# JaehaKim97/EDTR

Measured on AMD Instinct MI355X. Metric: restored 512x512 images/sec @ 4 denoise steps, higher is better.
Workload: dtype bf16; 1 GPU; EDTR-det s4 (sd21): vae_encode + q_sample(t=200) + 4 x (ControlNet+UNet) + vae_decode, batch 8/GPU of 512x512; global_batch=8, image_size=512, denoise_steps=4, parallelism=batch-sharded x1, graphs=True, batches_in_flight=2, precision=fast

## Files before the change

edtr_amd/csrc/lin320.hip:

```cpp
#include <stdlib.h>
#include <type_traits>
#include "common.h"

namespace {

constexpr int LK = 320;
constexpr int LKS = LK / 16;
constexpr int LBM = 128;
constexpr int LCH = 32;
constexpr int LCHB = LCH * LK * 2;
constexpr int LPITCH = 272;
constexpr int LVPITCH = 144;
constexpr int LSTGB = 64 * LVPITCH;
constexpr int L_STG = 2 * LCHB;
constexpr int L_CV = L_STG + 4 * LSTGB;
constexpr int L_LDS = L_CV + 4096;
static_assert(LSTGB >= 32 * LPITCH && 2 * L_LDS <= 160 * 1024, "LDS budget");

template <int N> __device__ __forceinline__ void lwait() {
    static_assert(N == 0 || N == 4 || N == 5 || N == 9, "lwait");
    if constexpr (N == 0) asm volatile("s_waitcnt vmcnt(0)" ::: "memory");
    else if constexpr (N == 4) asm volatile("s_waitcnt vmcnt(4)" ::: "memory");
    else if constexpr (N == 5) asm volatile("s_waitcnt vmcnt(5)" ::: "memory");
    else asm volatile("s_waitcnt vmcnt(9)" ::: "memory");
// ... 186 lines not shown
        case 2: return go(&lin320_kernel<T, true, false, false>);
        case 3: return go(&lin320_kernel<T, true, true, false>);
        case 4: return go(&lin320_kernel<T, false, false, true>);
        default: return go(&lin320_kernel<T, false, true, true>);
    }
}

int check_lin320(const edtr_lin320_params& p) {
    if (!p.x || !p.w || !p.out) return EDTR_E_NULL;
    if (p.dtype != EDTR_BF16 && p.dtype != EDTR_F16) return EDTR_E_DTYPE;
    if (p.K != LK || p.M <= 0 || p.N <= 0) return EDTR_E_SHAPE;
    if ((p.M % LBM) || (p.N % 64) || p.N > 1024) return EDTR_E_UNSUPPORTED;
    if (p.ldx < LK || (p.residual && p.ldr < p.N)) return EDTR_E_SHAPE;
    if ((p.ldx & 7) || (p.ldo & 7) || (p.residual && (p.ldr & 7))) return EDTR_E_ALIGN;
    if (!aligned16(p.x) || !aligned16(p.w) || !aligned16(p.out) || (p.residual && !aligned16(p.residual)) || (p.cvec && !aligned16(p.cvec))) return EDTR_E_ALIGN;
    if (p.x == p.out) return EDTR_E_UNSUPPORTED;
    if (p.gn_table) {
        if (p.ln || p.rows_per_image <= 0 || (p.rows_per_image % LBM) || (p.M % p.rows_per_image)) return EDTR_E_UNSUPPORTED;
        if (!aligned16(p.gn_table)) return EDTR_E_ALIGN;
    }
    if (p.vt_out) {
        if (p.residual || p.vt_col0 <= 0 || p.vt_col0 >= p.N || (p.vt_col0 & 63) || p.rows_per_image <= 0 || (p.rows_per_image & 31) ||
            (p.M % p.rows_per_image) || p.vt_ld < p.rows_per_image)
            return EDTR_E_UNSUPPORTED;
        if ((p.vt_ld & 7) || !aligned16(p.vt_out)) return EDTR_E_ALIGN;
        if (p.ldo < p.vt_col0) return EDTR_E_SHAPE;
    } else if (p.ldo < p.N) {
        return EDTR_E_SHAPE;
    }
    if ((int64_t)p.N * LK * 2 >= 0xF0000000LL) return EDTR_E_UNSUPPORTED;
    return EDTR_OK;
}

}

extern "C" int edtr_lin320(const edtr_lin320_params* pp, edtr_stream_t stream) {
    if (!pp) return EDTR_E_NULL;
    if (int e = check_lin320(*pp)) return e;
    hipStream_t s = static_cast<hipStream_t>(stream);
    return pp->dtype == EDTR_BF16 ? launch_lin320<BF16>(*pp, s) : launch_lin320<F16>(*pp, s);
}

extern "C" int edtr_lin320_plan(const edtr_lin320_params* pp) {
    if (!pp) return EDTR_E_NULL;
    return check_lin320(*pp);
}
```

edtr_amd/engine.py:

```python
from __future__ import annotations

import collections
import ctypes as ct
import math
import os
from dataclasses import dataclass
from typing import Dict, List, Optional, Sequence, Tuple

import torch

from . import lib as L
from . import ops
from .ops import Rec, round_up


class Arena:

    ALIGN = 256

    def __init__(self, device: torch.device, chunk_bytes: int = 1 << 28):
        self.device = device
        self.chunk_bytes = chunk_bytes
        self.chunks: List[torch.Tensor] = []
        self.free_lists: List[List[List[int]]] = []
# ... 225 lines not shown
            npad = packed.shape[0]
            c1 = packed[:, : w.shape[1]].float().sum(dim=1).contiguous()
            c2 = ops.pad_bias(w @ beta, npad).contiguous()
            self.cache[key] = (packed, ops.pad_bias(b, npad) if b is not None else None, c1, c2)
        packed, b, c1, c2 = self.cache[key]
        return packed, b, c1, c2

    def ffn(self, w1name: str, b1name: str, w2name: str, b2name: str, ln_prefix: str):
        key = ("ffn", w1name, w2name, ln_prefix)
        if key not in self.cache:
            w1p, b1p, c1, c2 = self.ln_fold("geglu", [w1name], [b1name], ln_prefix)
            cst = ops.pack_ffn_constants(c2 + b1p)
            w2p = ops.pack_ffn_w2(self._p(w2name).reshape(self.params[w2name].shape[0], -1), self.dtype)
            self.cache[key] = (w1p, w2p, cst, self._p(b2name).reshape(-1).contiguous())
        return self.cache[key]

    def lin320(self, names: Sequence[str], biases, ln_prefix: Optional[str], alpha: float, vt_col0: Optional[int] = None, vt_alpha: float = 1.0):
        names = tuple(names)
        key = ("lin320", names, tuple(biases) if biases else None, ln_prefix, float(alpha), vt_col0, float(vt_alpha))
        if key not in self.cache:
            w = torch.cat([self._p(n).reshape(self.params[n].shape[0], -1) for n in names], dim=0)
            cvec = None
            if biases:
                cvec = torch.cat([self._p(bn).reshape(-1) if bn else torch.zeros(self.params[n].shape[0], device=self.device)
                                  for n, bn in zip(names, biases)]).float()
            if ln_prefix is not None:
                gamma, beta = self._p(ln_prefix + "weight").reshape(-1), self._p(ln_prefix + "bias").reshape(-1)
                shift = float(alpha) * (w @ beta)
                if vt_col0 is not None:
                    shift[vt_col0:] *= float(vt_alpha) / float(alpha)
                cvec = shift if cvec is None else cvec + shift
                w = w * gamma[None, :]
            self.cache[key] = (ops.pack_lin320_w(w, self.dtype), cvec.contiguous() if cvec is not None else None)
        return self.cache[key]

    def raw(self, name: str) -> torch.Tensor:
        key = ("raw", name)
        if key not in self.cache:
            self.cache[key] = self._p(name).contiguous()
        return self.cache[key]

    def geglu(self, wname: str, bname: str):
        n, k = self.shape_of(wname)[0], self.shape_of(wname)[1]

        def build(parts):
            w = self._p(wname)
            perm = ops.geglu_perm(w.shape[0] // 2).to(self.device)
            return ops.pack_linear_weight(w[perm], self.dtype, parts=parts)

        ref = WRef(self, ("geglu", wname), build, (round_up(n, 8), round_up(k, 8)))
        key = ("geglu.bias", bname)
        if key not in self.cache:
            b = self._p(bname)
            self.cache[key] = b[ops.geglu_perm(b.shape[0] // 2).to(self.device)].contiguous()
        return ref, self.cache[key]

    def tensors(self) -> List[torch.Tensor]:
        out: List[torch.Tensor] = []
        seen = set()
        stores = [self] + [self._siblings[k] for k in sorted(self._siblings, key=str)]
        for st in stores:
            for key in sorted(st.cache, key=repr):
                val = st.cache[key]
                for t in (val if isinstance(val, (tuple, list)) else (val,)):
                    if isinstance(t, torch.Tensor) and t.data_ptr() not in seen:
                        seen.add(t.data_ptr())
# ... 450 lines not shown
        self.arena.free(tmp)
        return qk, vt, N

    def conv(self, x: Act, prefix: str, *, taps=9, stride=1, pad_tl=1, ups=False, rowvec=None, residual=None,
             out=None, out_f32=False, alpha=1.0, name=None, stats=False, feeds=None, mirror=False, gnp_into=None) -> Act:
        name = name or ("conv3x3" if taps == 9 else "conv1x1")
        w, bias = self.store.conv(prefix, cin_pad=x.C, bias_scale=alpha)
        N = w.shape[0]
        if taps == 9:
            LH, LW = (x.H * 2, x.W * 2) if ups else (x.H, x.W)
            pad_br = 1
            OH = (LH + pad_tl + pad_br - 3) // stride + 1
            OW = (LW + pad_tl + pad_br - 3) // stride + 1
            spatial = (x.H, x.W, OH, OW, stride, pad_tl, pad_tl, int(ups))
        else:
            OH, OW, spatial = x.H, x.W, None
        M = x.B * OH * OW
        parts = self.parts_for(name, M, N, taps * x.C)
        if parts == ops.PARTS_2W and (taps != 1 or x.C % 64):
            parts = 3
        if x.gn_in is not None:
            img8_ = taps == 9 and stride == 1 and pad_tl == 1 and not ups and (x.H, x.W) == (8, 8) and x.C % 64 == 0
            fusable = (taps == 9 and stride == 1 and pad_tl == 1 and not ups and not self.invariant
                       and (not self.hp or (x.t.dtype == self.dtype and parts == 1))
                       and ops.gn_in_conv_ok(x.B, x.H, x.W, x.C, N, ops.choose_splitk(M, N, taps * x.C, img8=img8_)[1], x.ld))
            if not fusable:
                if x.gn_apply is None:
                    raise RuntimeError(f"{name}: a deferred GroupNorm reached a convolution that cannot apply it")
                xn = x.gn_apply()
                y = self.conv(xn, prefix, taps=taps, stride=stride, pad_tl=pad_tl, ups=ups, rowvec=rowvec, residual=residual, out=out,
                              out_f32=out_f32, alpha=alpha, name=name, stats=stats, feeds=feeds, mirror=mirror, gnp_into=gnp_into)
                self.free(xn)
                return y
        a, tmp = x.t, None
        if self.hp:
            a, tmp, parts = self._operand(x.t, x.rows, x.C, parts)
            out_f32 = True if out is None else out.dtype == torch.float32
            if out is None and self.branch16 and feeds and self.feeds_parts(feeds, M) == 1:
                out_f32 = False
        Ce = ops.k_mult(parts) * x.C
        subpix = (ups and taps == 9 and stride == 1 and pad_tl == 1 and not self.invariant
                  and ops.subpixel_ok(x.H, x.W, Ce, N, x.B, a.stride(0)))
        if subpix:
            w, bias = self.store.conv_subpixel(prefix, cin_pad=x.C, bias_scale=alpha)
            spatial = spatial[:7] + (2,)
        wt = self._w(w, parts)
        m16 = None
        if out is None:
            out = self.new(M, N, torch.float32 if out_f32 else (self.dtype if self.hp else None))
            if mirror and self.mirrors_on and out_f32:
                m16 = self.add_mirror(out)
        elif self.mirrors_on and out_f32:
            m16 = self.mirror_view(out)
        img8 = taps == 9 and stride == 1 and pad_tl == 1 and not ups and (x.H, x.W) == (8, 8) and Ce % 64 == 0
        tile, splitk = ops.choose_splitk(M, N, taps * Ce, img8=img8)
        if self.invariant:
            tile, splitk = ops.invariant_tile(Ce, 0), 1
        if subpix:
            tile, splitk = 16, 1
        if x.gn_in is not None:
            if (taps != 9 or stride != 1 or pad_tl != 1 or ups or (self.hp and (a.dtype != self.dtype or parts != 1 or a is not x.t))
                    or not ops.gn_in_conv_ok(x.B, x.H, x.W, x.C, N, splitk, x.ld)):
                raise RuntimeError(f"{name}: a deferred GroupNorm reached a convolution that cannot apply it")
            tile = 0
        ws = self.arena.alloc((splitk * M * N,), torch.float32) if splitk > 1 else None
        gnp, gn_slot, into = None, 128, None
        self.gnp_into_done = False
        if stats and (self.hp or not out_f32) and out.stride(0) == N and ops.gn_fusable(M, N, Ce, OH * OW, splitk=splitk, invariant=self.invariant):
            gn_slot = ops.gn_slot_rows(OH * OW) if splitk > 1 else 128
            gnp = self.arena.alloc((M // gn_slot, N, 2), torch.float32)
        elif gnp_into is not None and not out_f32:
            into = self._gnp_into_args(gnp_into, M, N, Ce, OH * OW, splitk)
            self.gnp_into_done = into is not None
        res32 = residual is not None and residual.dtype == torch.float32
        self.prog.add(ops.make_igemm(
            dtype=self.dtype, a1=a, w=wt, out=out, taps=taps, M=M, N=N, C1=Ce, ld1=a.stride(0), ldw=wt.stride(0),
            ldc=out.stride(0), spatial=spatial, bias_n=bias, rowvec=rowvec,
            rowvec_ld=rowvec.stride(0) if rowvec is not None else 0, rows_per_image=OH * OW, residual=residual,
            ldr=residual.stride(0) if residual is not None else 0, residual_f32=res32, out_f32=out_f32, alpha=alpha, tile=tile,
            splitk=splitk, workspace=ws, name=name,
            **(into if into is not None else dict(gn_partial=gnp, gn_slot_rows=gn_slot if splitk > 1 else 0)),
            w_phase_stride=(N * wt.stride(0)) if subpix else 0,
            out16=m16, a_wrap=x.C if parts == ops.PARTS_2W else 0, a_gn=x.gn_in, a_gn_silu=x.gn_silu))
        self.arena.free(ws)
        self.arena.free(tmp)
        return Act(out, x.B, OH, OW, N, gnp, gn_slot=gn_slot)

    def conv128_out(self, x: Act, prefix: str, out_nchw: torch.Tensor, n_valid: int, alpha: float = 1.0, name="vae.conv_out") -> None:
        key = ("conv128_out", prefix, alpha)
        if key not in self.store.cache:
            w = self.store._p(prefix + "weight")
            self.store.cache[key] = (ops.pack_conv128_out_weight(w, self.dtype), ops.pad_bias(self.store._p(prefix + "bias") * alpha, 32))
        w, b = self.store.cache[key]
        self.prog.add(ops.make_conv128_out(dtype=self.dtype, x=x.t, ldx=x.ld, w=w, bias=b, out=out_nchw, B=x.B, H=x.H, W=x.W, n_valid=n_valid,
                                           gn_table=x.gn_in, alpha=alpha, name=name))

    def _gn_recs(self, x: Act, prefix: str, eps: float, silu: bool, sums: Optional[torch.Tensor], y: torch.Tensor,
                 sums_zeroed: bool = False, parts: int = 1, partial=None):
        gamma, beta = self.store.vec(prefix + "weight", x.C), self.store.vec(prefix + "bias", x.C)
        c_real = self.store.params[prefix + "weight"].numel()
        if c_real != x.C:
            raise ValueError(f"GroupNorm {prefix}: activation has {x.C} channels, parameter has {c_real}")
        in32 = x.t.dtype == torch.float32
        return ops.make_gn(dtype=(self.op_fmt(parts) if in32 else self.dtype) if self.hp else self.io, x=x.t, ldx=x.ld, B=x.B, HW=x.H * x.W, C=x.C,
                           sums=sums, gamma=gamma, beta=beta, eps=eps, silu=silu, y=y, ldy=y.stride(0), sums_zeroed=sums_zeroed,
                           partial=partial, tiles_per_image=x.gn_tiles)

    def _norm_out(self, rows: int, C: int, parts: int):
        if self.hp:
            t = self.arena.alloc((rows, parts * C), self.dtype)
            return t, OpN(t, C, parts)
        y = self.new(rows, C)
        return y, y

    def gn_deferrable(self, x: Act, conv_n: int, feeds=None) -> bool:
        if not conv_n or self.invariant or x.t.dtype == torch.float32:
            return False
        if self.hp and (conv_n < 0 or x.t.dtype != self.dtype or feeds is None or self.feeds_parts(feeds, x.rows) != 1
                        or os.environ.get("EDTR_GN_IN_CONV_HP", "1") == "0"):
            return False
# ... 230 lines not shown
```

edtr_amd/lib.py:

```python
from __future__ import annotations

import ctypes as C
import os
from typing import Optional

HERE = os.path.dirname(os.path.abspath(__file__))
LIB_PATH = os.environ.get("EDTR_AMD_LIB") or os.path.join(HERE, "libedtr_hip.so")

BF16, F16, F32_SPLIT, F32_H1, F32_H2, F32_H3 = 0, 1, 2, 3, 4, 5
ACT_NONE, ACT_GEGLU, ACT_SILU, ACT_GELU, ACT_LRELU = 0, 1, 2, 3, 4
SQDIFF_BLOCKS = 64
TILE_WINDOWS_MAX = 4096
RESIZE_BILINEAR, RESIZE_BICUBIC, RESIZE_AREA = 0, 1, 2
LOGITS_F32, LOGITS_F16, LOGITS_BF16 = 0, 1, 2
SEG_MAX_CLASSES = 32
NMS_MAX_BOXES = 32768
BOX_SHIFT, BOX_MUL, BOX_DIV, BOX_CLIP = 1, 2, 4, 8
COCO_MAX_DET, COCO_MAX_GT, COCO_MAX_LABELS, COCO_MAX_THRESHOLDS, COCO_KEEP = 1024, 1024, 256, 10, 100
CLS_MAX_CLASSES, CLS_MAX_KEEP, CLS_MAX_TOPK, CLS_FD_CHUNK, CLS_FD_MAX_ELEMS = 65536, 8, 4, 4096, 1 << 28
RPN_MAX_LEVELS, RPN_MAX_PRE_NMS, ROI_MAX_TAPS = 8, 4096, 64

DECLARED_SYMBOLS = [
    "edtr_abi_version", "edtr_error_string", "edtr_device_info", "edtr_igemm", "edtr_flash_attn64",
    "edtr_gn_stats", "edtr_gn_apply", "edtr_gn_finalize", "edtr_gn_table", "edtr_layernorm", "edtr_softmax_rows", "edtr_nchw_to_nhwc",
    "edtr_nhwc_to_nchw", "edtr_add", "edtr_timestep_embedding", "edtr_sampler_update", "edtr_axpby", "edtr_q_sample", "edtr_split3", "edtr_cast16",
    "edtr_tile_accumulate", "edtr_divide", "edtr_wavelet_level", "edtr_gn_pool", "edtr_copy3d_f32", "edtr_graph_begin", "edtr_graph_end", "edtr_graph_launch",
    "edtr_graph_destroy", "edtr_zero_bytes", "edtr_embed_tokens", "edtr_window_attn", "edtr_pixel_unshuffle", "edtr_swin_mlp", "edtr_swin_attn", "edtr_swin_layer", "edtr_conv64", "edtr_conv128_out",
    "edtr_split_operand", "edtr_sampler_update_indexed", "edtr_gaussian_sample", "edtr_add_mirror", "edtr_igemm_plan", "edtr_flash_attn512",
    "edtr_ffn", "edtr_ffn_plan", "edtr_add_stats", "edtr_lin320", "edtr_lin320_plan",
    "edtr_normal_fill", "edtr_q_sample_rng", "edtr_sampler_update_rng", "edtr_sampler_update_indexed_rng", "edtr_gaussian_sample_rng",
    "edtr_image_resize_u8", "edtr_image_ingest", "edtr_image_emit", "edtr_image_sqdiff",
    "edtr_image_resize_h_batch", "edtr_image_resize_ingest_batch", "edtr_image_emit_batch",
    "edtr_tile_gather", "edtr_tile_blend",
    "edtr_degrade_filter2d", "edtr_degrade_resize", "edtr_degrade_gaussian_noise", "edtr_degrade_jpeg",
    "edtr_degrade_poisson_noise", "edtr_degrade_sepblur", "edtr_degrade_usm_apply",
    "edtr_seg_confusion", "edtr_label_resize_nearest", "edtr_label_window", "edtr_label_colorize",
    "edtr_boxes_rank", "edtr_boxes_nms", "edtr_boxes_candidates", "edtr_boxes_filter_shift", "edtr_boxes_transform", "edtr_boxes_bilinear_scale",
    "edtr_coco_match",
    "edtr_cls_rank", "edtr_cls_fdist", "edtr_cls_commit", "edtr_cls_normalize", "edtr_cls_window",
    "edtr_rpn_anchors", "edtr_rpn_select", "edtr_rpn_candidates", "edtr_roi_align",
]


class IgemmParams(C.Structure):
    _fields_ = [
        ("dtype", C.c_int32), ("taps", C.c_int32), ("M", C.c_int32), ("N", C.c_int32), ("K", C.c_int32),
        ("n_valid", C.c_int32), ("Z", C.c_int32), ("zdiv", C.c_int32),
        ("a1", C.c_void_p), ("a2", C.c_void_p),
        ("C1", C.c_int32), ("C2", C.c_int32), ("ld1", C.c_int32), ("ld2", C.c_int32),
        ("a_zs_outer", C.c_int64), ("a_zs_inner", C.c_int64),
        ("IH", C.c_int32), ("IW", C.c_int32), ("OH", C.c_int32), ("OW", C.c_int32),
        ("stride", C.c_int32), ("pad_t", C.c_int32), ("pad_l", C.c_int32), ("upsample2x", C.c_int32),
        ("w", C.c_void_p), ("ldw", C.c_int32),
        ("w_zs_outer", C.c_int64), ("w_zs_inner", C.c_int64),
        ("alpha", C.c_float),
        ("bias_n", C.c_void_p), ("bias_m", C.c_void_p),
        ("rowvec", C.c_void_p), ("rowvec_ld", C.c_int32), ("rows_per_image", C.c_int32),
        ("act", C.c_int32),
        ("residual", C.c_void_p), ("ldr", C.c_int32),
        ("out", C.c_void_p), ("ldc", C.c_int32), ("out_f32", C.c_int32),
        ("o_zs_outer", C.c_int64), ("o_zs_inner", C.c_int64),
        ("tile", C.c_int32), ("splitk", C.c_int32),
# ... 43 lines not shown
class SwinMlpParams(C.Structure):
    _fields_ = [
        ("dtype", C.c_int32), ("rows", C.c_int32), ("C", C.c_int32), ("hidden", C.c_int32), ("c_valid", C.c_int32),
        ("eps", C.c_float),
        ("x", C.c_void_p), ("ldx", C.c_int32),
        ("w1", C.c_void_p), ("w2", C.c_void_p),
        ("c1", C.c_void_p), ("c2b", C.c_void_p), ("b2", C.c_void_p),
        ("out", C.c_void_p), ("ldo", C.c_int32),
        ("row_stats", C.c_void_p),
    ]


class FfnParams(C.Structure):
    _fields_ = [
        ("dtype", C.c_int32), ("M", C.c_int32), ("D", C.c_int32), ("H", C.c_int32),
        ("eps", C.c_float),
        ("x", C.c_void_p), ("ldx", C.c_int32),
        ("w1", C.c_void_p), ("w2", C.c_void_p),
        ("cst", C.c_void_p), ("b2", C.c_void_p),
        ("out", C.c_void_p), ("ldo", C.c_int32),
    ]


class Lin320Params(C.Structure):
    _fields_ = [
        ("dtype", C.c_int32), ("M", C.c_int32), ("N", C.c_int32), ("K", C.c_int32),
        ("ln", C.c_int32), ("eps", C.c_float), ("alpha", C.c_float),
        ("x", C.c_void_p), ("ldx", C.c_int32),
        ("w", C.c_void_p), ("cvec", C.c_void_p),
        ("residual", C.c_void_p), ("ldr", C.c_int32),
        ("out", C.c_void_p), ("ldo", C.c_int32),
        ("vt_out", C.c_void_p), ("vt_col0", C.c_int32), ("vt_ld", C.c_int32), ("vt_alpha", C.c_float), ("rows_per_image", C.c_int32),
        ("gn_table", C.c_void_p),
    ]


class SwinAttnParams(C.Structure):
    _fields_ = [
        ("dtype", C.c_int32), ("B", C.c_int32), ("H", C.c_int32), ("W", C.c_int32),
        ("heads", C.c_int32), ("head_dim", C.c_int32), ("shift", C.c_int32),
        ("C", C.c_int32), ("c_valid", C.c_int32),
        ("eps", C.c_float),
        ("x", C.c_void_p), ("ldx", C.c_int32),
        ("wqkv", C.c_void_p), ("wproj", C.c_void_p),
        ("c1", C.c_void_p), ("c2b", C.c_void_p), ("bproj", C.c_void_p),
        ("bias", C.c_void_p), ("labels", C.c_void_p),
        ("out", C.c_void_p), ("ldo", C.c_int32),
    ]


class Conv64Params(C.Structure):
    _fields_ = [
        ("dtype", C.c_int32), ("B", C.c_int32), ("H", C.c_int32), ("W", C.c_int32),
        ("upsample2x", C.c_int32),
        ("x", C.c_void_p), ("ldx", C.c_int32),
        ("w", C.c_void_p), ("bias", C.c_void_p),
        ("act", C.c_int32), ("act_slope", C.c_float), ("alpha", C.c_float),
        ("out", C.c_void_p), ("ldo", C.c_int32),
        ("out_nchw_f32", C.c_int32), ("n_valid", C.c_int32),
    ]


class Conv128OutParams(C.Structure):
    _fields_ = [
        ("dtype", C.c_int32), ("B", C.c_int32), ("H", C.c_int32), ("W", C.c_int32),
        ("x", C.c_void_p), ("ldx", C.c_int32),
# ... 66 lines not shown
    lib.edtr_q_sample.argtypes = [vp, vp, vp, vp, vp, i32, vp, i32, i64, vp]
    lib.edtr_split3.argtypes = [i32, vp, i64, i32, i64, i32, vp, i64, vp]
    lib.edtr_cast16.argtypes = [i32, vp, i64, i32, i64, vp, i64, vp]
    lib.edtr_split_operand.argtypes = [i32, vp, i64, i32, i64, i32, vp, i64, vp]
    lib.edtr_sampler_update_indexed.argtypes = [vp, vp, vp, vp, vp, i32, vp, vp, i32, i64, vp]
    lib.edtr_gaussian_sample.argtypes = [vp, i32, vp, vp, i32, i32, i64, f32, vp]
    lib.edtr_tile_accumulate.argtypes = [vp, vp, vp, vp, i32, i32, i32, i32, i32, i32, i32, i32, vp]
    lib.edtr_divide.argtypes = [vp, vp, vp, i64, vp]
    lib.edtr_wavelet_level.argtypes = [vp, vp, vp, i32, i32, i32, i32, vp]
    lib.edtr_gn_pool.argtypes = [vp, vp, vp, i32, i32, vp]
    lib.edtr_copy3d_f32.argtypes = [vp, i64, i64, vp, i64, i64, i32, i32, i32, vp]
    lib.edtr_graph_begin.argtypes = [vp]
    lib.edtr_graph_end.argtypes = [vp, C.POINTER(vp)]
    lib.edtr_graph_launch.argtypes = [vp, vp]
    lib.edtr_graph_destroy.argtypes = [vp]
    for name in DECLARED_SYMBOLS:
        fn = getattr(lib, name)
        if name not in ("edtr_error_string",):
            fn.restype = i32
    lib.edtr_zero_bytes.argtypes = [vp, i64, vp]
    lib.edtr_embed_tokens.argtypes = [i32, vp, vp, vp, i32, i32, i32, i32, vp, i32, vp]
    lib.edtr_window_attn.argtypes = [C.POINTER(WindowAttnParams), vp]
    lib.edtr_pixel_unshuffle.argtypes = [i32, vp, i32, i32, i32, i32, i32, vp, f32, vp, i32, i32, vp]
    lib.edtr_swin_mlp.argtypes = [C.POINTER(SwinMlpParams), vp]
    lib.edtr_swin_attn.argtypes = [C.POINTER(SwinAttnParams), vp]
    lib.edtr_conv64.argtypes = [C.POINTER(Conv64Params), vp]
    lib.edtr_conv128_out.argtypes = [C.POINTER(Conv128OutParams), vp]
    lib.edtr_swin_layer.argtypes = [C.POINTER(SwinAttnParams), C.POINTER(SwinMlpParams), vp]
    lib.edtr_add_stats.argtypes = [i32, vp, i32, vp, i32, vp, i32, i64, i32, vp, i32, i32, vp]
    lib.edtr_ffn.argtypes = [C.POINTER(FfnParams), vp]
    lib.edtr_ffn_plan.argtypes = [C.POINTER(FfnParams)]
    lib.edtr_lin320.argtypes = [C.POINTER(Lin320Params), vp]
    lib.edtr_lin320_plan.argtypes = [C.POINTER(Lin320Params)]
    u64 = C.c_uint64
    lib.edtr_normal_fill.argtypes = [vp, i32, i64, u64, vp, i64, i32, i64, vp]
    lib.edtr_q_sample_rng.argtypes = [vp, vp, vp, vp, i32, vp, i32, i64, u64, vp, i64, vp]
    lib.edtr_sampler_update_rng.argtypes = [vp, vp, f32, f32, f32, f32, f32, vp, vp, i32, i64, u64, vp, i64, i64, vp]
    lib.edtr_sampler_update_indexed_rng.argtypes = [vp, vp, vp, vp, i32, vp, vp, i32, i64, u64, vp, i64, vp]
    lib.edtr_gaussian_sample_rng.argtypes = [vp, i32, vp, i32, i32, i64, f32, u64, vp, i64, vp]
    lib.edtr_image_resize_u8.argtypes = [vp, i32, i32, i32, vp, i32, i32, vp, vp, i32, vp, vp, i32, vp, vp]
    lib.edtr_image_ingest.argtypes = [i32, vp, i32, i32, i32, vp, i32, i32, i32, i32, i32, vp, vp]
    lib.edtr_image_emit.argtypes = [vp, i32, i32, i32, i32, i32, vp, i32, i32, vp]
    lib.edtr_image_sqdiff.argtypes = [vp, vp, i32, i32, i32, i32, vp, i32, i32, vp, vp, vp]
    lib.edtr_image_resize_h_batch.argtypes = [C.POINTER(ImageDesc), vp, i32, i32, vp, i64, vp]
    lib.edtr_image_resize_ingest_batch.argtypes = [C.POINTER(ImageDesc), vp, i32, i32, vp, i64, vp, i32, i32, i32, i32, vp, vp]
    lib.edtr_image_emit_batch.argtypes = [vp, i32, i32, i32, i32, C.POINTER(i64), vp, i32, vp, i64, vp]
    lib.edtr_tile_gather.argtypes = [vp, i32, i32, i32, i32, C.POINTER(i32), vp, i32, i32, i32, vp, vp]
    lib.edtr_tile_blend.argtypes = [vp, vp, C.POINTER(i32), vp, i32, i32, i32, vp, i32, i32, i32, i32, vp]
    lib.edtr_degrade_filter2d.argtypes = [vp, vp, i32, i32, i32, i32, vp, i32, i32, vp]
    lib.edtr_degrade_resize.argtypes = [vp, vp, i32, i32, i32, i32, i32, i32, i32, vp]
    lib.edtr_degrade_gaussian_noise.argtypes = [vp, vp, vp, i32, i32, i32, i32, C.POINTER(f32), vp, C.POINTER(i32), vp, u64, vp, i64, i64, i32, vp]
    lib.edtr_degrade_jpeg.argtypes = [vp, vp, i32, i32, i32, i32, C.POINTER(f32), vp, vp, vp, vp]
    lib.edtr_degrade_poisson_noise.argtypes = [vp, vp, vp, i32, i32, i32, i32, C.POINTER(f32), vp, C.POINTER(i32), vp, vp, vp, vp, vp, u64, vp, i64, i64, i32, vp]
    lib.edtr_degrade_sepblur.argtypes = [vp, vp, vp, i32, i32, i32, i32, vp, i32, f32, vp]
    lib.edtr_degrade_usm_apply.argtypes = [vp, vp, vp, vp, i32, i32, i32, i32, f32, vp]
    lib.edtr_seg_confusion.argtypes = [i32, vp, vp, i32, i32, i32, i32, C.POINTER(i32), vp, vp, vp, i32, vp]
    lib.edtr_label_resize_nearest.argtypes = [vp, i32, i32, i32, vp, i32, i32, vp, vp, vp]
    lib.edtr_label_window.argtypes = [vp, i32, i32, i32, vp, i32, i32, i32, i32, i32, i32, i32, vp]
    lib.edtr_label_colorize.argtypes = [vp, i32, i32, i32, vp, vp, vp]
    lib.edtr_boxes_rank.argtypes = [vp, i32, vp, vp]
    lib.edtr_boxes_nms.argtypes = [vp, vp, vp, i32, i32, f32, vp, vp, vp, i32, vp, vp]
    lib.edtr_boxes_candidates.argtypes = [vp, vp, vp, i32, i32, f32, f32, f32, f32, C.POINTER(f32), f32, vp, vp, vp, vp, vp, vp, vp, vp, vp]
    lib.edtr_boxes_filter_shift.argtypes = [vp, vp, vp, i32, f32, f32, f32, vp, vp, vp, vp, i32, vp]
    lib.edtr_boxes_transform.argtypes = [vp, vp, i32, i32, f32, f32, f32, f32, f32, f32, vp]
    lib.edtr_boxes_bilinear_scale.argtypes = [vp, vp, i32, i32, i32, i32, i32, f32, f32, vp]
    lib.edtr_coco_match.argtypes = [vp, vp, vp, i32, vp, vp, vp, vp, vp, i32, i32, i32, i32, vp, i32, vp, vp, vp, vp, vp, vp, vp, vp, i32, vp, vp, vp, vp, i32, vp]
# ... 20 lines not shown
```

edtr_amd/ops.py:

```python
from __future__ import annotations

import ctypes as ct
import os
from typing import Optional, Sequence, Tuple

import torch

from . import lib as L

F32S = "f32_split"
F32H = {1: "f32_h1", 2: "f32_h2", 3: "f32_h3"}
MIXED = "f32_mixed"
PARTS_2W = 4
_DT = {torch.bfloat16: L.BF16, torch.float16: L.F16, F32S: L.F32_SPLIT, F32H[1]: L.F32_H1, F32H[2]: L.F32_H2, F32H[3]: L.F32_H3}


def dt_code(dtype: torch.dtype) -> int:
    try:
        return _DT[dtype]
    except KeyError:
        raise TypeError(f"libedtr_hip stores activations as bfloat16 or float16, got {dtype}")


def stream_ptr() -> int:
# ... 271 lines not shown
LIN320_K, LIN320_ROWS = 320, 128


def lin320_ok(M: int, N: int, K: int, ln: bool = False) -> bool:
    if os.environ.get("EDTR_LIN320", "1") == "0" or K != LIN320_K or M <= 0 or M % LIN320_ROWS or N % 64 or N > 1024:
        return False
    env = os.environ.get("EDTR_LIN320_MIN_ROWS")
    return M >= (int(env) if env else (16384 if (ln and N <= 320) else 32768))


def pack_lin320_w(w: torch.Tensor, dtype: torch.dtype) -> torch.Tensor:
    n, k = w.shape
    assert k == LIN320_K and n % 32 == 0
    w16 = w.to(dtype).reshape(n // 32, 32, k // 16, 2, 8)
    return w16.permute(0, 2, 3, 1, 4).contiguous().reshape(-1)


def make_lin320(*, dtype, x, ldx, M, N, w, cvec=None, alpha=1.0, ln=False, eps=1e-5, residual=None, ldr=0, out, ldo, vt_out=None, vt_col0=0,
                vt_ld=0, vt_alpha=1.0, rows_per_image=0, gn_table=None, name="lin320") -> Rec:
    p = L.Lin320Params()
    p.dtype, p.M, p.N, p.K, p.ln, p.eps, p.alpha = dt_code(dtype), M, N, LIN320_K, int(ln), eps, alpha
    p.x, p.ldx, p.w, p.cvec = ptr(x), ldx, ptr(w), ptr(cvec)
    p.residual, p.ldr, p.out, p.ldo = ptr(residual), ldr, ptr(out), ldo
    p.vt_out, p.vt_col0, p.vt_ld, p.vt_alpha, p.rows_per_image = ptr(vt_out), vt_col0, vt_ld, vt_alpha, rows_per_image
    p.gn_table = ptr(gn_table)
    flops = 2.0 * M * N * LIN320_K
    nbytes = 2.0 * M * (LIN320_K + N * (2 if residual is not None else 1)) + 2.0 * N * LIN320_K
    rec = Rec(L.load().edtr_lin320, (ct.byref(p),), (p, x, w, cvec, residual, out, vt_out, gn_table), name, flops, nbytes)
    rec.tag = (f"lin320 M{M} N{N}" + (" ln" if ln else "") + (" gnin" if gn_table is not None else "") + (" res" if residual is not None else "")
               + (" vT" if vt_out is not None else ""))
    return rec


def make_swin_layer(attn: Rec, mlp: Rec, name="swin.layer") -> Rec:
    pa, pm = attn.keep[0], mlp.keep[0]
    return Rec(L.load().edtr_swin_layer, (ct.byref(pa), ct.byref(pm)), (attn.keep, mlp.keep), name, attn.flops + mlp.flops,
               attn.bytes + mlp.bytes - 4.0 * pa.B * pa.H * pa.W * SWIN_MLP_C)


def pack_conv64_weight(w: torch.Tensor, dtype: torch.dtype) -> torch.Tensor:
    co, ci, kh, kw = w.shape
    assert (kh, kw) == (3, 3) and co <= 64 and ci <= 64
    full = torch.zeros((9, 64, 8, 8), dtype=torch.float32, device=w.device)
    full.reshape(9, 64, 64)[:, :co, :ci] = w.permute(2, 3, 0, 1).reshape(9, co, ci)
    n = torch.arange(64, device=w.device)[:, None]
    c = torch.arange(8, device=w.device)[None, :]
    img = torch.empty_like(full)
    img[:, n, c ^ ((n >> 1) & 7)] = full[:, n, c]
    return img.to(dtype).reshape(-1).contiguous()


def pack_conv128_out_weight(w: torch.Tensor, dtype: torch.dtype) -> torch.Tensor:
    co, ci, kh, kw = w.shape
    assert (kh, kw) == (3, 3) and co <= 32 and ci == 128
    full = torch.zeros((9, 32, 16, 8), dtype=torch.float32, device=w.device)
    full.reshape(9, 32, 128)[:, :co] = w.permute(2, 3, 0, 1).reshape(9, co, ci)
    n = torch.arange(32, device=w.device)[:, None]
    c = torch.arange(16, device=w.device)[None, :]
    img = torch.empty_like(full)
    img[:, n, c ^ (n & 15)] = full[:, n, c]
    return img.to(dtype).reshape(-1).contiguous()


def conv128_out_ok(H: int, W: int, cin: int, cout: int) -> bool:
    return os.environ.get("EDTR_CONV128_OUT", "1") != "0" and cin == 128 and cout <= 4 and H % 16 == 0 and W % 16 == 0

# ... 693 lines not shown
```

include/edtr_hip.h:

```cpp
#ifndef EDTR_HIP_H
#define EDTR_HIP_H

#include <stdint.h>

#ifdef __cplusplus
extern "C" {
#endif

#define EDTR_ABI_VERSION 10

enum edtr_dtype {
    EDTR_BF16 = 0, EDTR_F16 = 1,
    EDTR_F32_SPLIT = 2,
    EDTR_F32_H1 = 3, EDTR_F32_H2 = 4, EDTR_F32_H3 = 5
};

enum edtr_error {
    EDTR_OK = 0,
    EDTR_E_NULL = -1,
    EDTR_E_SHAPE = -2,
    EDTR_E_ALIGN = -3,
    EDTR_E_DTYPE = -4,
    EDTR_E_UNSUPPORTED = -5
};
// ... 136 lines not shown

int edtr_swin_layer(const edtr_swin_attn_params* attn, const edtr_swin_mlp_params* mlp, edtr_stream_t stream);

typedef struct edtr_ffn_params {
    int32_t dtype;
    int32_t M, D, H;
    float eps;
    const void* x; int32_t ldx;
    const void* w1; const void* w2;
    const float* cst; const float* b2;
    void* out; int32_t ldo;
} edtr_ffn_params;

int edtr_ffn(const edtr_ffn_params* p, edtr_stream_t stream);
int edtr_ffn_plan(const edtr_ffn_params* p);

typedef struct edtr_lin320_params {
    int32_t dtype;
    int32_t M, N, K;
    int32_t ln; float eps;
    float alpha;
    const void* x; int32_t ldx;
    const void* w;
    const float* cvec;
    const void* residual; int32_t ldr;
    void* out; int32_t ldo;
    void* vt_out; int32_t vt_col0; int32_t vt_ld; float vt_alpha; int32_t rows_per_image;
    const float* gn_table;
} edtr_lin320_params;

int edtr_lin320(const edtr_lin320_params* p, edtr_stream_t stream);
int edtr_lin320_plan(const edtr_lin320_params* p);

typedef struct edtr_conv64_params {
    int32_t dtype;
    int32_t B, H, W;
    int32_t upsample2x;
    const void* x; int32_t ldx;
    const void* w;
    const float* bias;
    int32_t act; float act_slope; float alpha;
    void* out; int32_t ldo;
    int32_t out_nchw_f32, n_valid;
} edtr_conv64_params;

int edtr_conv64(const edtr_conv64_params* p, edtr_stream_t stream);

typedef struct edtr_conv128_out_params {
    int32_t dtype;
    int32_t B, H, W;
    const void* x; int32_t ldx;
    const float* gn_table;
    const void* w;
    const float* bias;
    float alpha;
    void* out; int32_t n_valid;
} edtr_conv128_out_params;

int edtr_conv128_out(const edtr_conv128_out_params* p, edtr_stream_t stream);

int edtr_softmax_rows(int dtype, const float* s, int64_t rows, int cols, int64_t ld_s, void* p,
                      int64_t ld_p, int cols_pad, edtr_stream_t stream);

int edtr_embed_tokens(int dtype, const int64_t* tokens, const float* table, const float* pos, int rows, int L, int D,
                      int vocab, void* out, int ld, edtr_stream_t stream);
int edtr_zero_bytes(void* ptr, int64_t bytes, edtr_stream_t stream);
// ... 204 lines not shown
```

Measured before the change: 119.4 images/s.

## Add specialized 3x3 conv kernel for 8x8 spatial UNet layers

Adds a dedicated conv8 kernel for 3x3 stride-1 convolutions on 8x8 feature maps, where each block holds a whole padded 10x10 image patch (one or two images) in LDS. It computes 32 output channels, splits K across the four waves and reduces them through LDS. Weights are prepacked per 32-channel slice and register-pipelined several chunks ahead. The epilogue fuses bias, timestep rowvec, residual and GroupNorm partial statistics. It targets the poorly parallelized small-M implicit-GEMM convs in the lowest UNet/ControlNet resolution, at the cost of a special path restricted to fast mode and to grids that fit the CU count.

```diff
diff --git a/edtr_amd/csrc/conv8.inc b/edtr_amd/csrc/conv8.inc
--- /dev/null
+++ b/edtr_amd/csrc/conv8.inc
@@ -0,0 +1,243 @@
+constexpr int C8_NS = 32;
+constexpr int C8_PATCH = 100 * 128;
+constexpr int C8_CHUNKB = 36 * 1024;
+constexpr int C8_LDS1 = 4 * 8192;
+constexpr int C8_AHEAD = 4;
+static_assert(2 * C8_PATCH <= C8_LDS1, "the partial tiles cover the patch buffers");
+
+template <int V> using C8I = std::integral_constant<int, V>;
+
+__device__ __forceinline__ void c8_barrier() {
+    asm volatile("s_waitcnt lgkmcnt(0)" ::: "memory");
+    __builtin_amdgcn_s_barrier();
+    asm volatile("" ::: "memory");
+}
+
+template <typename T, bool RES, int G>
+__global__ void __launch_bounds__(256, G == 1 ? 2 : 1) conv8_kernel(const edtr_conv8_params p) {
+    __shared__ __attribute__((aligned(16))) char smem[G * C8_LDS1];
+    constexpr int PB = G * C8_PATCH;
+    const int tid = threadIdx.x, lane = tid & 63, wave = __builtin_amdgcn_readfirstlane(tid >> 6);
+    const int l31 = lane & 31, lh = lane >> 5;
+    const int nchunk = p.Cin >> 6;
+    int bid = blockIdx.x;
+    {
+        const int nblk = gridDim.x, q = nblk >> 3, r = nblk & 7, x = bid & 7, j = bid >> 3;
+        bid = (x < r ? x * (q + 1) : r * (q + 1) + (x - r) * q) + j;
+    }
+    const int ngroup = p.B / G;
+    const int slice = bid / ngroup, img0 = (bid - slice * ngroup) * G, n0 = slice * C8_NS;
+
+    for (int i = tid; i < 2 * PB / 16; i += 256) *reinterpret_cast<U4*>(smem + 16 * i) = zero16();
+
+    const int sc = tid & 7;
+    int st[2];
+    uint32_t xoff[G][2];
+#pragma unroll
+    for (int j = 0; j < 2; ++j) {
+        const int pix = (tid >> 3) + 32 * j, py = (pix >> 3) + 1, px = (pix & 7) + 1;
+        st[j] = (py * 10 + px) * 128 + ((sc ^ (((px >> 1) & 1) | ((py & 3) << 1))) << 4);
+#pragma unroll
+        for (int g = 0; g < G; ++g) xoff[g][j] = (uint32_t)(((img0 + g) * 64 + pix) * p.ldx + sc * 8) * 2u;
+    }
+    const char* const xb = static_cast<const char*>(p.x);
+    int a_rd[9];
+#pragma unroll
+    for (int t = 0; t < 9; ++t) {
+        const int py = (l31 >> 3) + t / 3, px = (l31 & 7) + t % 3;
+        a_rd[t] = (py * 10 + px) * 128 + (((2 * wave + lh) ^ (((px >> 1) & 1) | ((py & 3) << 1))) << 4);
+    }
+    const char* const wb = static_cast<const char*>(p.w) + (size_t)slice * nchunk * C8_CHUNKB + wave * 9216 + lane * 16;
+
+    U4 wr[4][9], xr[2][G][2];
+    auto load_w = [&](auto Ic, int c) {
+        constexpr int I = decltype(Ic)::value;
+#pragma unroll
+        for (int t = 0; t < 9; ++t) wr[I][t] = ldg16(wb + (size_t)c * C8_CHUNKB + t * 1024);
+    };
+    auto load_x = [&](auto Ic, int c) {
+        constexpr int I = decltype(Ic)::value;
+#pragma unroll
+        for (int g = 0; g < G; ++g)
+#pragma unroll
+            for (int j = 0; j < 2; ++j) xr[I][g][j] = ldg16(xb + xoff[g][j] + c * 128);
+    };
+    auto store_x = [&](auto Ic, char* buf) {
+        constexpr int I = decltype(Ic)::value;
+#pragma unroll
+        for (int g = 0; g < G; ++g)
+#pragma unroll
+            for (int j = 0; j < 2; ++j) *reinterpret_cast<U4*>(buf + g * C8_PATCH + st[j]) = xr[I][g][j];
+    };
+    f32x16 acc[G][2];
+#pragma unroll
+    for (int g = 0; g < G; ++g)
+#pragma unroll
+        for (int r = 0; r < 16; ++r) { acc[g][0][r] = 0.0f; acc[g][1][r] = 0.0f; }
+
+    const int last = nchunk - 1;
+    load_x(C8I<0>{}, 0);
+    load_x(C8I<1>{}, last < 1 ? last : 1);
+    load_w(C8I<0>{}, 0);
+    load_w(C8I<1>{}, last < 1 ? last : 1);
+    load_w(C8I<2>{}, last < 2 ? last : 2);
+    c8_barrier();
+    store_x(C8I<0>{}, smem);
+    c8_barrier();
+
+    auto step = [&](auto Ic, int c) {
+        constexpr int I = decltype(Ic)::value;
+        load_x(C8I<(I & 1)>{}, c + 2 < last ? c + 2 : last);
+        __builtin_amdgcn_sched_barrier(0);
+        load_w(C8I<(I + 3) % 4>{}, c + 3 < last ? c + 3 : last);
+        __builtin_amdgcn_sched_barrier(0);
+        const char* pa = smem + (c & 1) * PB;
+        U4 a[C8_AHEAD][G][2];
+#pragma unroll
+        for (int t = 0; t < C8_AHEAD; ++t)
+#pragma unroll
+            for (int g = 0; g < G; ++g) {
+                a[t][g][0] = *reinterpret_cast<const U4*>(pa + g * C8_PATCH + a_rd[t]);
+                a[t][g][1] = *reinterpret_cast<const U4*>(pa + g * C8_PATCH + a_rd[t] + 40 * 128);
+            }
+        __builtin_amdgcn_sched_barrier(0);
+#pragma unroll
+        for (int t = 0; t < 9; ++t) {
+#pragma unroll
+            for (int g = 0; g < G; ++g) {
+                acc[g][0] = T::mfma(a[t % C8_AHEAD][g][0], wr[I][t], acc[g][0]);
+                acc[g][1] = T::mfma(a[t % C8_AHEAD][g][1], wr[I][t], acc[g][1]);
+            }
+            if (t + C8_AHEAD < 9) {
+#pragma unroll
+                for (int g = 0; g < G; ++g) {
+                    a[t % C8_AHEAD][g][0] = *reinterpret_cast<const U4*>(pa + g * C8_PATCH + a_rd[t + C8_AHEAD]);
+                    a[t % C8_AHEAD][g][1] = *reinterpret_cast<const U4*>(pa + g * C8_PATCH + a_rd[t + C8_AHEAD] + 40 * 128);
+                }
+            }
+            __builtin_amdgcn_sched_barrier(0);
+        }
+        store_x(C8I<((I + 1) & 1)>{}, smem + ((c + 1) & 1) * PB);
+        c8_barrier();
+    };
+    int c = 0;
+#pragma unroll 1
+    for (; c + 4 <= nchunk; c += 4) {
+        step(C8I<0>{}, c);
+        step(C8I<1>{}, c + 1);
+        step(C8I<2>{}, c + 2);
+        step(C8I<3>{}, c + 3);
+    }
+    if (c < nchunk) step(C8I<0>{}, c);
+    if (c + 1 < nchunk) step(C8I<1>{}, c + 1);
+    if (c + 2 < nchunk) step(C8I<2>{}, c + 2);
+
+#pragma unroll
+    for (int g = 0; g < G; ++g) {
+        float* red = reinterpret_cast<float*>(smem + g * C8_LDS1) + wave * 2048 + lane;
+#pragma unroll
+        for (int r = 0; r < 16; ++r) { red[r * 64] = acc[g][0][r]; red[(16 + r) * 64] = acc[g][1][r]; }
+    }
+    const int pix = tid >> 2, ng = tid & 3, n = n0 + 8 * ng;
+    U4 rv[G];
+#pragma unroll
+    for (int g = 0; g < G; ++g) {
+        rv[g] = zero16();
+        if constexpr (RES) rv[g] = ldg16(static_cast<const uint16_t*>(p.residual) + ((int64_t)(img0 + g) * 64 + pix) * p.ldr + n);
+    }
+    f32x4 b0 = f32x4{0.0f, 0.0f, 0.0f, 0.0f}, b1 = b0;
+    if (p.bias_n) { b0 = *reinterpret_cast<const f32x4*>(p.bias_n + n); b1 = *reinterpret_cast<const f32x4*>(p.bias_n + n + 4); }
+    c8_barrier();
+    float f[G][8];
+#pragma unroll
+    for (int g = 0; g < G; ++g) {
+        f32x4 t0 = f32x4{0.0f, 0.0f, 0.0f, 0.0f}, t1 = t0;
+        if (p.rowvec) {
+            const float* tv = p.rowvec + (int64_t)(img0 + g) * p.rowvec_ld + n;
+            t0 = *reinterpret_cast<const f32x4*>(tv); t1 = *reinterpret_cast<const f32x4*>(tv + 4);
+        }
+        const int q = pix & 31, jr = (pix >> 5) * 16 + (q & 3) + 4 * (q >> 3);
+        const float* src = reinterpret_cast<const float*>(smem + g * C8_LDS1) + jr * 64 + ((q >> 2) & 1) * 32 + 8 * ng;
+#pragma unroll
+        for (int e = 0; e < 8; ++e) f[g][e] = 0.0f;
+#pragma unroll
+        for (int w = 0; w < 4; ++w) {
+            const f32x4 v0 = *reinterpret_cast<const f32x4*>(src + w * 2048), v1 = *reinterpret_cast<const f32x4*>(src + w * 2048 + 4);
+#pragma unroll
+            for (int e = 0; e < 4; ++e) { f[g][e] += v0[e]; f[g][e + 4] += v1[e]; }
+        }
+#pragma unroll
+        for (int e = 0; e < 4; ++e) { f[g][e] = f[g][e] * p.alpha + b0[e] + t0[e]; f[g][e + 4] = f[g][e + 4] * p.alpha + b1[e] + t1[e]; }
+        if constexpr (RES) {
+            float rf[8];
+            unpack8<T>(rv[g], rf);
+#pragma unroll
+            for (int e = 0; e < 8; ++e) f[g][e] += rf[e];
+        }
+        stg16(static_cast<uint16_t*>(p.out) + ((int64_t)(img0 + g) * 64 + pix) * p.ldc + n, pack8<T>(f[g]));
+    }
+    if (p.gn_partial) {
+        c8_barrier();
+        float* gsc = reinterpret_cast<float*>(smem);
+#pragma unroll
+        for (int g = 0; g < G; ++g) {
+            float gs[8], gq[8];
+#pragma unroll
+            for (int e = 0; e < 8; ++e) { gs[e] = f[g][e]; gq[e] = f[g][e] * f[g][e]; }
+#pragma unroll
+            for (int o = 4; o < 64; o <<= 1)
+#pragma unroll
+                for (int e = 0; e < 8; ++e) { gs[e] += __shfl_xor(gs[e], o, 64); gq[e] += __shfl_xor(gq[e], o, 64); }
+            if (lane < 4) {
+#pragma unroll
+                for (int e = 0; e < 8; ++e) {
+                    gsc[((g * 4 + wave) * 32 + 8 * lane + e) * 2] = gs[e];
+                    gsc[((g * 4 + wave) * 32 + 8 * lane + e) * 2 + 1] = gq[e];
+                }
+            }
+        }
+        c8_barrier();
+        if (tid < C8_NS * G) {
+            const int g = tid >> 5, col = tid & 31;
+            float s = 0.0f, q = 0.0f;
+#pragma unroll
+            for (int w = 0; w < 4; ++w) { s += gsc[((g * 4 + w) * 32 + col) * 2]; q += gsc[((g * 4 + w) * 32 + col) * 2 + 1]; }
+            const int gld = p.gn_ld > 0 ? p.gn_ld : p.N;
+            float* dst = p.gn_partial + ((int64_t)(img0 + g) * gld + n0 + col) * 2;
+            dst[0] = s;
+            dst[1] = q;
+        }
+    }
+}
+
+int check_conv8(const edtr_conv8_params& p) {
+    if (!p.x || !p.w || !p.out) return EDTR_E_NULL;
+    if (p.dtype != EDTR_BF16 && p.dtype != EDTR_F16) return EDTR_E_DTYPE;
+    if (p.B <= 0 || p.Cin <= 0 || p.N <= 0) return EDTR_E_SHAPE;
+    if (p.H != 8 || p.W != 8 || (p.Cin & 63) || (p.N % C8_NS)) return EDTR_E_UNSUPPORTED;
+    if (p.ldx < p.Cin || p.ldc < p.N || (p.residual && p.ldr < p.N) || (p.rowvec && p.rowvec_ld < p.N) || (p.gn_partial && p.gn_ld > 0 && p.gn_ld < p.N))
+        return EDTR_E_SHAPE;
+    if ((p.ldx & 7) || (p.ldc & 7) || (p.residual && (p.ldr & 7)) || (p.rowvec && (p.rowvec_ld & 3))) return EDTR_E_ALIGN;
+    if (!aligned16(p.x) || !aligned16(p.w) || !aligned16(p.out) || (p.residual && !aligned16(p.residual)) || (p.bias_n && !aligned16(p.bias_n)) ||
+        (p.rowvec && !aligned16(p.rowvec)) || (p.gn_partial && (reinterpret_cast<uintptr_t>(p.gn_partial) & 7u)))
+        return EDTR_E_ALIGN;
+    if (p.x == p.out) return EDTR_E_UNSUPPORTED;
+    if ((int64_t)p.B * 64 * p.ldx * 2 >= 0xF0000000LL || (int64_t)p.B * (p.N / C8_NS) >= 0x7FFFFFFFLL) return EDTR_E_UNSUPPORTED;
+    return EDTR_OK;
+}
+
+template <typename T>
+int launch_conv8(const edtr_conv8_params& p, hipStream_t stream) {
+    const int nslice = p.N / C8_NS;
+    const bool two = (p.B & 1) == 0 && p.B * nslice > edtr_cu_count();
+    const dim3 grid((unsigned)((two ? p.B / 2 : p.B) * nslice)), block(256);
+    if (two) {
+        if (p.residual) hipLaunchKernelGGL((conv8_kernel<T, true, 2>), grid, block, 0, stream, p);
+        else hipLaunchKernelGGL((conv8_kernel<T, false, 2>), grid, block, 0, stream, p);
+    } else {
+        if (p.residual) hipLaunchKernelGGL((conv8_kernel<T, true, 1>), grid, block, 0, stream, p);
+        else hipLaunchKernelGGL((conv8_kernel<T, false, 1>), grid, block, 0, stream, p);
+    }
+    EDTR_LAUNCH_CHECK();
+    return EDTR_OK;
+}
diff --git a/edtr_amd/csrc/lin320.hip b/edtr_amd/csrc/lin320.hip
--- a/edtr_amd/csrc/lin320.hip
+++ b/edtr_amd/csrc/lin320.hip
@@ -242,6 +242,8 @@
     return EDTR_OK;
 }
 
+#include "conv8.inc"
+
 }
 
 extern "C" int edtr_lin320(const edtr_lin320_params* pp, edtr_stream_t stream) {
@@ -255,3 +257,15 @@
     if (!pp) return EDTR_E_NULL;
     return check_lin320(*pp);
 }
+
+extern "C" int edtr_conv8(const edtr_conv8_params* pp, edtr_stream_t stream) {
+    if (!pp) return EDTR_E_NULL;
+    if (int e = check_conv8(*pp)) return e;
+    hipStream_t s = static_cast<hipStream_t>(stream);
+    return pp->dtype == EDTR_BF16 ? launch_conv8<BF16>(*pp, s) : launch_conv8<F16>(*pp, s);
+}
+
+extern "C" int edtr_conv8_plan(const edtr_conv8_params* pp) {
+    if (!pp) return EDTR_E_NULL;
+    return check_conv8(*pp);
+}
diff --git a/edtr_amd/engine.py b/edtr_amd/engine.py
--- a/edtr_amd/engine.py
+++ b/edtr_amd/engine.py
@@ -281,6 +281,14 @@
                 cvec = shift if cvec is None else cvec + shift
                 w = w * gamma[None, :]
             self.cache[key] = (ops.pack_lin320_w(w, self.dtype), cvec.contiguous() if cvec is not None else None)
+        return self.cache[key]
+
+    def conv8(self, prefix: str) -> torch.Tensor:
+        if self.dtype in (ops.F32S, ops.MIXED):
+            raise ValueError("edtr_conv8 is a fast-mode launch (the parity modes keep edtr_igemm)")
+        key = ("conv8", prefix)
+        if key not in self.cache:
+            self.cache[key] = ops.pack_conv8_w(self._p(prefix + "weight"), self.dtype)
         return self.cache[key]
 
     def raw(self, name: str) -> torch.Tensor:
@@ -797,6 +805,9 @@
                               out_f32=out_f32, alpha=alpha, name=name, stats=stats, feeds=feeds, mirror=mirror, gnp_into=gnp_into)
                 self.free(xn)
                 return y
+        if (taps == 9 and stride == 1 and pad_tl == 1 and not ups and not self.hp and not self.invariant and parts == 1 and x.gn_in is None
+                and not out_f32 and self.conv8_ok(x, prefix, N, rowvec, residual, out)):
+            return self._conv8(x, prefix, N, bias, rowvec=rowvec, residual=residual, out=out, alpha=alpha, name=name, stats=stats, gnp_into=gnp_into)
         a, tmp = x.t, None
         if self.hp:
             a, tmp, parts = self._operand(x.t, x.rows, x.C, parts)
@@ -851,6 +862,36 @@
         self.arena.free(tmp)
         return Act(out, x.B, OH, OW, N, gnp, gn_slot=gn_slot)
 
+    def conv8_ok(self, x: Act, prefix: str, N: int, rowvec=None, residual=None, out=None) -> bool:
+        if not ops.conv8_ok(x.B, x.H, x.W, x.C, N, x.ld, hp=self.hp, invariant=self.invariant) or x.t.dtype != self.dtype:
+            return False
+        if self.store.shape_of(prefix + "weight") != (N, x.C, 3, 3):
+            return False
+        for t in (residual, out):
+            if t is not None and (t.dtype != self.dtype or t.stride(0) % 8 or t.data_ptr() % 16):
+                return False
+        return rowvec is None or (rowvec.dtype == torch.float32 and rowvec.stride(0) % 4 == 0 and rowvec.data_ptr() % 16 == 0)
+
+    def _conv8(self, x: Act, prefix: str, N: int, bias, *, rowvec, residual, out, alpha, name, stats, gnp_into) -> Act:
+        M = x.rows
+        if out is None:
+            out = self.new(M, N)
+        gnp, part, gld = None, None, 0
+        self.gnp_into_done = False
+        fus = ops.gn_fusable(M, N, x.C, 64, splitk=2)
+        if stats and fus and out.stride(0) == N:
+            gnp = self.arena.alloc((x.B, N, 2), torch.float32)
+            part, gld = gnp, N
+        elif gnp_into is not None and fus and gnp_into[2] == 64:
+            buf, col, _ = gnp_into
+            part, gld = buf.reshape(-1)[2 * col:], buf.shape[1]
+            self.gnp_into_done = True
+        self.prog.add(ops.make_conv8(dtype=self.dtype, x=x.t, ldx=x.ld, B=x.B, Cin=x.C, N=N, w=self.store.conv8(prefix), out=out, ldc=out.stride(0),
+                                     alpha=alpha, bias_n=bias, rowvec=rowvec, rowvec_ld=rowvec.stride(0) if rowvec is not None else 0,
+                                     residual=residual, ldr=residual.stride(0) if residual is not None else 0, gn_partial=part, gn_ld=gld,
+                                     name=name))
+        return Act(out, x.B, 8, 8, N, gnp, gn_slot=64)
+
     def conv128_out(self, x: Act, prefix: str, out_nchw: torch.Tensor, n_valid: int, alpha: float = 1.0, name="vae.conv_out") -> None:
         key = ("conv128_out", prefix, alpha)
         if key not in self.store.cache:
diff --git a/edtr_amd/lib.py b/edtr_amd/lib.py
--- a/edtr_amd/lib.py
+++ b/edtr_amd/lib.py
@@ -27,7 +27,7 @@
     "edtr_tile_accumulate", "edtr_divide", "edtr_wavelet_level", "edtr_gn_pool", "edtr_copy3d_f32", "edtr_graph_begin", "edtr_graph_end", "edtr_graph_launch",
     "edtr_graph_destroy", "edtr_zero_bytes", "edtr_embed_tokens", "edtr_window_attn", "edtr_pixel_unshuffle", "edtr_swin_mlp", "edtr_swin_attn", "edtr_swin_layer", "edtr_conv64", "edtr_conv128_out",
     "edtr_split_operand", "edtr_sampler_update_indexed", "edtr_gaussian_sample", "edtr_add_mirror", "edtr_igemm_plan", "edtr_flash_attn512",
-    "edtr_ffn", "edtr_ffn_plan", "edtr_add_stats", "edtr_lin320", "edtr_lin320_plan",
+    "edtr_ffn", "edtr_ffn_plan", "edtr_add_stats", "edtr_lin320", "edtr_lin320_plan", "edtr_conv8", "edtr_conv8_plan",
     "edtr_normal_fill", "edtr_q_sample_rng", "edtr_sampler_update_rng", "edtr_sampler_update_indexed_rng", "edtr_gaussian_sample_rng",
     "edtr_image_resize_u8", "edtr_image_ingest", "edtr_image_emit", "edtr_image_sqdiff",
     "edtr_image_resize_h_batch", "edtr_image_resize_ingest_batch", "edtr_image_emit_batch",
@@ -137,6 +137,20 @@
         ("out", C.c_void_p), ("ldo", C.c_int32),
         ("vt_out", C.c_void_p), ("vt_col0", C.c_int32), ("vt_ld", C.c_int32), ("vt_alpha", C.c_float), ("rows_per_image", C.c_int32),
         ("gn_table", C.c_void_p),
+    ]
+
+
+class Conv8Params(C.Structure):
+    _fields_ = [
+        ("dtype", C.c_int32), ("B", C.c_int32), ("H", C.c_int32), ("W", C.c_int32), ("Cin", C.c_int32), ("N", C.c_int32),
+        ("x", C.c_void_p), ("ldx", C.c_int32),
+        ("w", C.c_void_p),
+        ("alpha", C.c_float),
+        ("bias_n", C.c_void_p),
+        ("rowvec", C.c_void_p), ("rowvec_ld", C.c_int32),
+        ("residual", C.c_void_p), ("ldr", C.c_int32),
+        ("out", C.c_void_p), ("ldc", C.c_int32),
+        ("gn_partial", C.c_void_p), ("gn_ld", C.c_int32),
     ]
 
 
@@ -269,6 +283,8 @@
     lib.edtr_ffn_plan.argtypes = [C.POINTER(FfnParams)]
     lib.edtr_lin320.argtypes = [C.POINTER(Lin320Params), vp]
     lib.edtr_lin320_plan.argtypes = [C.POINTER(Lin320Params)]
+    lib.edtr_conv8.argtypes = [C.POINTER(Conv8Params), vp]
+    lib.edtr_conv8_plan.argtypes = [C.POINTER(Conv8Params)]
     u64 = C.c_uint64
     lib.edtr_normal_fill.argtypes = [vp, i32, i64, u64, vp, i64, i32, i64, vp]
     lib.edtr_q_sample_rng.argtypes = [vp, vp, vp, vp, i32, vp, i32, i64, u64, vp, i64, vp]
diff --git a/edtr_amd/ops.py b/edtr_amd/ops.py
--- a/edtr_amd/ops.py
+++ b/edtr_amd/ops.py
@@ -327,6 +327,60 @@
     return rec
 
 
+CONV8_SLICE = 32
+_CUS: dict = {}
+
+
+def cu_count() -> int:
+    if "n" not in _CUS:
+        n = ct.c_int32(0)
+        try:
+            ok = L.load().edtr_device_info(ct.byref(n), None, None, 0) == 1 and n.value > 0
+        except (RuntimeError, OSError):
+            ok = False
+        _CUS["n"] = n.value if ok else 256
+    return _CUS["n"]
+
+
+CONV8_PAIRED_MAX_CIN = 1280
+
+
+def conv8_ok(B: int, H: int, W: int, C: int, N: int, ld: int = 0, hp: bool = False, invariant: bool = False) -> bool:
+    if os.environ.get("EDTR_CONV8", "1") == "0" or hp or invariant:
+        return False
+    if (H, W) != (8, 8) or C <= 0 or C % 64 or N <= 0 or N % CONV8_SLICE or B <= 0 or (ld or C) % 8:
+        return False
+    if B * 64 * (ld or C) * 2 >= 0xF0000000 or B < int(os.environ.get("EDTR_CONV8_MIN_IMAGES", "1")):
+        return False
+    cus, per_image = cu_count(), N // CONV8_SLICE
+    if B * per_image <= cus:
+        return True
+    return B % 2 == 0 and (B // 2) * per_image <= cus and C <= CONV8_PAIRED_MAX_CIN
+
+
+def pack_conv8_w(w: torch.Tensor, dtype: torch.dtype) -> torch.Tensor:
+    n, ci, kh, kw = w.shape
+    assert (kh, kw) == (3, 3) and n % CONV8_SLICE == 0 and ci % 64 == 0
+    w16 = w.to(dtype).reshape(n // 32, 32, ci // 64, 4, 2, 8, 9)
+    return w16.permute(0, 2, 3, 6, 4, 1, 5).contiguous().reshape(-1)
+
+
+def make_conv8(*, dtype, x, ldx, B, Cin, N, w, out, ldc, alpha=1.0, bias_n=None, rowvec=None, rowvec_ld=0, residual=None, ldr=0,
+               gn_partial=None, gn_ld=0, H=8, W=8, name="conv8") -> Rec:
+    p = L.Conv8Params()
+    p.dtype, p.B, p.H, p.W, p.Cin, p.N = dt_code(dtype), B, H, W, Cin, N
+    p.x, p.ldx, p.w, p.alpha = ptr(x), ldx, ptr(w), alpha
+    p.bias_n, p.rowvec, p.rowvec_ld = ptr(bias_n), ptr(rowvec), rowvec_ld
+    p.residual, p.ldr, p.out, p.ldc = ptr(residual), ldr, ptr(out), ldc
+    p.gn_partial, p.gn_ld = ptr(gn_partial), int(gn_ld)
+    M, K = B * H * W, 9 * Cin
+    flops = 2.0 * M * N * K
+    nbytes = 2.0 * M * Cin + 2.0 * N * K + 2.0 * M * N * (2 if residual is not None else 1)
+    rec = Rec(L.load().edtr_conv8, (ct.byref(p),), (p, x, w, bias_n, rowvec, residual, out, gn_partial), name, flops, nbytes)
+    rec.tag = f"conv8 M{M} N{N} K{K}" + (" gnp" if gn_partial is not None else "") + (" res" if residual is not None else "")
+    return rec
+
+
 def make_swin_layer(attn: Rec, mlp: Rec, name="swin.layer") -> Rec:
     pa, pm = attn.keep[0], mlp.keep[0]
     return Rec(L.load().edtr_swin_layer, (ct.byref(pa), ct.byref(pm)), (attn.keep, mlp.keep), name, attn.flops + mlp.flops,
diff --git a/include/edtr_hip.h b/include/edtr_hip.h
--- a/include/edtr_hip.h
+++ b/include/edtr_hip.h
@@ -192,6 +192,22 @@
 int edtr_lin320(const edtr_lin320_params* p, edtr_stream_t stream);
 int edtr_lin320_plan(const edtr_lin320_params* p);
 
+typedef struct edtr_conv8_params {
+    int32_t dtype;
+    int32_t B, H, W, Cin, N;
+    const void* x; int32_t ldx;
+    const void* w;
+    float alpha;
+    const float* bias_n;
+    const float* rowvec; int32_t rowvec_ld;
+    const void* residual; int32_t ldr;
+    void* out; int32_t ldc;
+    float* gn_partial; int32_t gn_ld;
+} edtr_conv8_params;
+
+int edtr_conv8(const edtr_conv8_params* p, edtr_stream_t stream);
+int edtr_conv8_plan(const edtr_conv8_params* p);
+
 typedef struct edtr_conv64_params {
     int32_t dtype;
     int32_t B, H, W;
```

Result: no change. 120.3 images/s (median of 6 runs) (+0.7%).
